# gabeur/mmt

Hardware: AMD Instinct MI355X
Metric: video-text pairs/sec (fwd+bwd+Adam), MSRVTT 7-expert d512 L4 (higher is better)
Workload: dtype bf16; 1 GPU; configs[1]: MSRVTT jsfusion shape, 7 experts x 30 tokens, d512, L4, H4, I3072, batch 32/GPU, dropout 0.1, train mode, Adam; text tower replaced by synthetic (B,768) vectors; global_batch=32, seq_len=218, parallelism=dp1, hip_graphs=True, inputs=resident in HBM, input_slots=8, input_format=dense fp32 dict, text_tower=synthetic, grad_sync=single, grad_wire_dtype=fp32, grad_algo=allreduce, comm_log=False, collectives_captured=False, dense_rows=6976, full=False

## Files before the change

### mmt_amd/csrc/gemm.hip

```cpp
#include "mmt_common.h"
#include "../../include/mmt_hip.h"

#define BK 64

template <int R>
__device__ __forceinline__ void stage_nt(const bf16_t* __restrict__ G, int64_t ld, int row0, int k0,
                                         bf16_t* lds_tile, int wave, int lane) {
#pragma unroll
  for (int i = 0; i < R / 32; ++i) {
    const int rbase = (wave * (R / 32) + i) * 8;
    const int r = rbase + (lane >> 3);
    const int c = (lane & 7) ^ (r & 7);
    const bf16_t* src = G + (int64_t)(row0 + r) * ld + k0 + c * 8;
    __builtin_amdgcn_global_load_lds(GLB_PTR(src), LDS_PTR(lds_tile + rbase * BK), 16, 0, 0);
  }
}

template <int BM, int BN, int EPI>
__global__ __launch_bounds__(256, 2) void gemm_nt_kernel(
    const bf16_t* __restrict__ A, int64_t lda, const bf16_t* __restrict__ B, int64_t ldb,
    void* __restrict__ Cout, int64_t ldc, int M, int N, int K, MmtEpilogue epi,
    const int32_t* __restrict__ n_rows_dev) {
  constexpr int MI = BM / 32, NI = BN / 32;
  __shared__ __attribute__((aligned(16))) bf16_t smem[2 * (BM + BN) * BK];
// ... 234 lines not shown
      const int k2 = k0 + wn * 64 + j * 16 + lg * 4;
      *(f32x4*)(out + (int64_t)n * K2 + k2) = acc[i][j];
    }
  }
}

__device__ __forceinline__ void tr_frag_issue(u32x2& lo, u32x2& hi, unsigned addr) {
  asm volatile("ds_read_b64_tr_b16 %0, %1" : "=v"(lo) : "v"(addr));
  asm volatile("ds_read_b64_tr_b16 %0, %1 offset:4096" : "=v"(hi) : "v"(addr));
}
__device__ __forceinline__ unsigned tr_frag_offset(int ks, int colbase, int lane) {
  const int t = lane & 15, g = lane >> 4;
  const int col = colbase + 4 * (t & 3);
  const int r0 = ks * 32 + 4 * g + (t >> 2);
  const int ch = col >> 3, w = col & 7;
  return (unsigned)((r0 * 128 + ((ch ^ ((r0 & 7) << 1)) << 3) + w) * 2);
}
#define TR_TIE4(x) "+v"(x[0]), "+v"(x[1]), "+v"(x[2]), "+v"(x[3])
__device__ __forceinline__ bf16x8_t tr_join(const u32x2& lo, const u32x2& hi) {
  const u32x4 v = {lo[0], lo[1], hi[0], hi[1]};
  return __builtin_bit_cast(bf16x8_t, v);
}

#ifdef MMT_GEMM2_INSTR
__device__ long long* g_wgrad_dbg = nullptr;
extern "C" int mmt_debug_set_wgrad_buffer(void* p) {
  return (int)hipMemcpyToSymbol(HIP_SYMBOL(g_wgrad_dbg), &p, sizeof(p));
}
#define WTICK(acc) do { const long long tn_ = clock64(); acc += tn_ - tp; tp = tn_; } while (0)
#else
#define WTICK(acc) do {} while (0)
#endif

__global__ __launch_bounds__(512) void wgrad_phased_kernel(MmtWgradGroup g) {
  extern __shared__ __attribute__((aligned(16))) unsigned char wg_smem[];
#ifdef MMT_GEMM2_INSTR
  const long long t_entry = clock64();
#endif
  bf16_t* smem = (bf16_t*)wg_smem;
  const int id = xcd_remap(blockIdx.x, gridDim.x);
  int p = 0;
#pragma unroll 1
  for (int q = 1; q < g.count; ++q)
    if (id >= g.item[q].tile_begin) p = q;
  const MmtWgradItem& it = g.item[p];
  const bf16_t* __restrict__ A = (const bf16_t*)it.A;
  const bf16_t* __restrict__ B = (const bf16_t*)it.B;
  const int64_t lda = it.lda, ldb = it.ldb;
  const int nsplit = it.splits > 1 ? it.splits : 1;
  const int tile = (id - it.tile_begin) / nsplit, split = (id - it.tile_begin) % nsplit;
  const int tiles_k = it.K2 / 128;
  int tn, tk;
  {
    const int PN = it.reserved2 >> 16, PK = it.reserved2 & 0xffff;
    if (PN > 0 && PK > 0) {
      const int per = PN * PK, patches_k = tiles_k / PK;
      const int patch = tile / per, within = tile % per;
      tn = (patch / patches_k) * PN + within / PK;
      tk = (patch % patches_k) * PK + within % PK;
    } else {
      tn = tile / tiles_k;
      tk = tile % tiles_k;
    }
  }
  const int n0 = tn * 128, k0 = tk * 128;
  const int nrows = it.reserved > 0 ? it.reserved
                    : it.n_rows_dev ? min(*it.n_rows_dev, g.rows)
                                    : (g.n_rows_dev ? min(*g.n_rows_dev, g.rows) : g.rows);
  const int units_all = (nrows + 63) / 64;
  const int per_split = (units_all + nsplit - 1) / nsplit;
  const int u0 = split * per_split;
  const int units = max(0, min(units_all, u0 + per_split) - u0);

  const int tid = threadIdx.x, lane = tid & 63, wave8 = tid >> 6;
  const int kg = wave8 >> 2, wave = wave8 & 3;
  const int wk = wave >> 1, wt = wave & 1;
  const int li = lane & 15, lg = lane >> 4;
// ... 224 lines not shown
  constexpr int kWgrad3MinRows = 2048, kWgrad3MinTiles = 192;
  {
    int t3 = 0;
    bool ok = h.rows >= kWgrad3MinRows;
    for (int q = 0; q < h.count && ok; ++q) {
      const MmtWgradItem& it = h.item[q];
      ok = it.A && it.B && it.out && it.N > 0 && it.K2 > 0 && it.N % 256 == 0 && it.K2 % 256 == 0 && it.splits <= 1 &&
           !(it.lda % 8) && !(it.ldb % 8) && !((uintptr_t)it.A & 15) && !((uintptr_t)it.B & 15) && !((uintptr_t)it.out & 15) &&
           it.lda >= 256 && it.ldb >= 256;
      t3 += (it.N / 256) * (it.K2 / 256);
    }
    if (ok && t3 >= kWgrad3MinTiles) {
      int tb = 0;
      for (int q = 0; q < h.count; ++q) {
        MmtWgradItem& it = h.item[q];
        if (it.N_out <= 0 || it.N_out > it.N) it.N_out = it.N;
        if (it.K2_out <= 0 || it.K2_out > it.K2) it.K2_out = it.K2;
        if (it.ldo <= 0) it.ldo = it.K2_out;
        it.tile_begin = tb;
        tb += (it.N / 256) * (it.K2 / 256);
      }
      return mmt_wgrad3_launch(h, tb, (hipStream_t)stream);
    }
  }
  for (int q = 0; q < h.count; ++q) {
    MmtWgradItem& it = h.item[q];
    if (!it.A || !it.B || !it.out || it.N <= 0 || it.K2 <= 0 || it.N % 128 || it.K2 % 128) return MMT_ERR_ARG;
    if ((it.lda % 8) || (it.ldb % 8) || ((uintptr_t)it.A & 15) || ((uintptr_t)it.B & 15) || ((uintptr_t)it.out & 15))
      return MMT_ERR_ALIGN;
    if (it.N_out <= 0 || it.N_out > it.N) it.N_out = it.N;
    if (it.K2_out <= 0 || it.K2_out > it.K2) it.K2_out = it.K2;
    if (it.ldo <= 0) it.ldo = it.K2_out;
    if (it.splits > 1 && (!it.slab || (it.bias_out && !it.bias_slab))) return MMT_ERR_ARG;
    it.tile_begin = tiles;
    tiles += (it.N / 128) * (it.K2 / 128) * (it.splits > 1 ? it.splits : 1);
    {
      const int tn_all = it.N / 128, tk_all = it.K2 / 128;
      int pn = 1, pk = 1;
      for (int c = 1; c <= 8; ++c)
        if (tn_all % c == 0) pn = c;
      for (int c = 1; c <= 32 / pn; ++c)
        if (tk_all % c == 0) pk = c;
      it.reserved2 = (pn << 16) | pk;
    }
  }
  constexpr int lds = 36 * 256 * 16;
  static bool configured = false;
  if (!configured) {
    hipError_t rc = hipFuncSetAttribute((const void*)wgrad_phased_kernel, hipFuncAttributeMaxDynamicSharedMemorySize, lds);
    if (rc != hipSuccess) return (int)rc;
    configured = true;
  }
  hipLaunchKernelGGL(wgrad_phased_kernel, dim3(tiles), dim3(512), lds, (hipStream_t)stream, h);
  return (int)hipGetLastError();
}

__global__ void reduce_slabs_kernel(const float* __restrict__ ws, int splits, int64_t count4,
                                    float* __restrict__ out, int accumulate) {
  for (int64_t i = blockIdx.x * (int64_t)blockDim.x + threadIdx.x; i < count4;
       i += (int64_t)gridDim.x * blockDim.x) {
    f32x4 s = ((const f32x4*)ws)[i];
    for (int k = 1; k < splits; ++k) s += ((const f32x4*)ws)[k * count4 + i];
    if (accumulate) s += ((const f32x4*)out)[i];
    ((f32x4*)out)[i] = s;
  }
}
// ... 151 lines not shown
```

### mmt_amd/csrc/gemm2.hip

```cpp
#include "mmt_common.h"
#include "../../include/mmt_hip.h"
#include "gemm_epi.h"

#define BK 64
template <int ROWS, int NW>
__device__ __forceinline__ void stage2(const bf16_t* __restrict__ G, int64_t ld, int row0, int row_max, int k0,
                                       bf16_t* lds_tile, int wave, int lane) {
  constexpr int PER = ROWS / 8 / NW;
#pragma unroll
  for (int i = 0; i < PER; ++i) {
    const int rbase = (wave * PER + i) * 8;
    const int r = rbase + (lane >> 3);
    const int c = (lane & 7) ^ ((r >> 1) & 7);
    const int gr = min(row0 + r, row_max);
    const bf16_t* src = G + (int64_t)gr * ld + k0 + c * 8;
    __builtin_amdgcn_global_load_lds(GLB_PTR(src), LDS_PTR(lds_tile + rbase * BK), 16, 0, 0);
  }
}

template <int BN> __device__ __forceinline__ int swz_kn(int r) {
  return BN == 128 ? (((r & 7) << 1) | ((r >> 3) & 1)) : ((r >> 1) & 7);
}
template <int BN, int NW>
__device__ __forceinline__ void stage2_kn(const bf16_t* __restrict__ G, int64_t ld, int k0, int n0, bf16_t* lds_tile,
// ... 5 lines not shown
    const int rbase = (wave * PER + i) * RPI;
    const int r = rbase + lane / CHN;
    const int c = (lane % CHN) ^ swz_kn<BN>(r);
    const bf16_t* src = G + (int64_t)(k0 + r) * ld + n0 + c * 8;
    __builtin_amdgcn_global_load_lds(GLB_PTR(src), LDS_PTR(lds_tile + rbase * BN), 16, 0, 0);
  }
}
template <int BN>
__device__ __forceinline__ bf16x8_t frag_kn(const bf16_t* tile, int kk, int colbase, int lane) {
  const int t = lane & 15;
  const int col = colbase + ((lane >> 4) & 1) * 16 + 4 * (t & 3);
  const int r0 = kk * 16 + (lane >> 5) * 8 + (t >> 2), r1 = r0 + 4;
  const int ch = col >> 3, w = col & 7;
  const bf16_t* p0 = tile + r0 * BN + ((ch ^ swz_kn<BN>(r0)) << 3) + w;
  const bf16_t* p1 = tile + r1 * BN + ((ch ^ swz_kn<BN>(r1)) << 3) + w;
  bf16x4_t lo = __builtin_amdgcn_ds_read_tr16_b64_v4bf16((__attribute__((address_space(3))) bf16x4_t*)LDS_PTR(p0));
  bf16x4_t hi = __builtin_amdgcn_ds_read_tr16_b64_v4bf16((__attribute__((address_space(3))) bf16x4_t*)LDS_PTR(p1));
  return __builtin_shufflevector(lo, hi, 0, 1, 2, 3, 4, 5, 6, 7);
}

template <int N>
__device__ __forceinline__ void wait_vmcnt() {
  asm volatile("s_waitcnt vmcnt(%0)" ::"n"(N) : "memory");
}

template <int BM, int BN, int WGM, int WGN, int NS, int EPI, bool BKN = false, bool PH = false>
__device__ __forceinline__ void gemm2_body(
    const bf16_t* __restrict__ A, int64_t lda, const bf16_t* __restrict__ B, int64_t ldb,
    void* __restrict__ Cout, int64_t ldc, int M, int N, int K, const MmtEpilogue& epi,
    const int32_t* __restrict__ n_rows_dev, const int bid, const int nblk) {
  constexpr int GW = WGM * WGN;
  constexpr int NW = PH ? 2 * GW : GW, NT = NW * 64, WTM = BM / WGM, WTN = BN / WGN, MI = WTM / 32, NJ = WTN / 32;
  static_assert(!PH || NS == 4, "the phased loop runs on a four-deep ring");
  constexpr bool STAG = !PH && NW == 8 && NS >= 3;
#ifdef MMT_GEMM2_INSTR
  const long long t_entry = clock64(), w_entry = wall_clock64();
#endif
  extern __shared__ __attribute__((aligned(16))) unsigned char smem_raw[];
  bf16_t* smem = (bf16_t*)smem_raw;

  const int tiles_n = N / BN;
  const int nrows = n_rows_dev ? *n_rows_dev : M;
  const int tid = threadIdx.x;
  const int live_tiles = min(nblk, ((min(nrows, M) + BM - 1) / BM) * tiles_n);
  if (bid >= live_tiles) {
    if constexpr (EPI == MMT_EPI_DGELU) {
      if (epi.colsum && BM >= 128 && bid < ((M + BM - 1) / BM) * tiles_n) {
        const int dm0 = (bid / tiles_n) * BM, dn0 = (bid % tiles_n) * BN;
        for (int h = 0; h < BM / 128; ++h)
          if (dm0 + h * 128 < M && tid < BN) epi.colsum[(int64_t)(dm0 / 128 + h) * N + dn0 + tid] = 0.f;
      }
    }
    return;
  }
  const int id = xcd_remap(bid, live_tiles);
  int tm, tn;
  if (tiles_n * BN >= 1024) {
    constexpr int GROUP = 8;
    const int tile_rows = live_tiles / tiles_n;
    const int band = id / (GROUP * tiles_n), first = band * GROUP;
    const int rows_here = min(GROUP, tile_rows - first);
    const int within = id - band * GROUP * tiles_n;
    tm = first + within % rows_here;
    tn = within / rows_here;
  } else {
    tm = id / tiles_n;
// ... 36 lines not shown
      stage2<BM, NW>(A, lda, m0, amax, s0 * BK, smem + s0 * STAGE, wave, lane);
      if constexpr (BKN) stage2_kn<BN, NW>(B, ldb, s0 * BK, n0, smem + s0 * STAGE + BM * BK, wave, lane);
      else stage2<BN, NW>(B, ldb, n0, bmax, s0 * BK, smem + s0 * STAGE + BM * BK, wave, lane);
    }
  }
  int aoff[MI], boff[NJ], asw[MI], bsw[NJ];
#pragma unroll
  for (int i = 0; i < MI; ++i) {
    const int r = wm * WTM + i * 32 + l31;
    aoff[i] = r * BK; asw[i] = (r >> 1) & 7;
  }
#pragma unroll
  for (int j = 0; j < NJ; ++j) {
    const int r = wn * WTN + j * 32 + l31;
    boff[j] = BM * BK + r * BK; bsw[j] = (r >> 1) & 7;
  }
  int cur = 0;
#ifdef MMT_GEMM2_INSTR
  long long t_wait = 0, t_bar = 0, t_issue = 0, t_comp = 0, t0 = clock64(), tp = t0;
#define TICK(acc) do { const long long tn_ = clock64(); acc += tn_ - tp; tp = tn_; } while (0)
#else
#define TICK(acc) do {} while (0)
#endif
  for (int kt = 0; kt < KT; ++kt) {
    bool do_issue = false;
    int nxt = 0;
    if constexpr (PH) {
      const bool mine = (kt & 1) == kg;
      if (mine) {
        if (kt + 2 < KT) wait_vmcnt<L>();
        else wait_vmcnt<0>();
      }
      TICK(t_wait);
      asm volatile("" ::: "memory");
      __builtin_amdgcn_s_barrier();
      asm volatile("" ::: "memory");
      TICK(t_bar);
      cur = kt % NS;
      if (!mine) {
        issue_ph(kt + NS - 1);
        TICK(t_issue);
        continue;
      }
    } else {
    const int ahead = min(KT - kt - 1, NS - 2);
    if (NS >= 4 && ahead >= 2) wait_vmcnt<2 * L>();
    else if (NS >= 3 && ahead >= 1) wait_vmcnt<L>();
    else wait_vmcnt<0>();
    TICK(t_wait);
    __builtin_amdgcn_s_barrier();
    asm volatile("" ::: "memory");
    TICK(t_bar);
    nxt = cur + NS - 1;
    if (nxt >= NS) nxt -= NS;
    do_issue = kt + NS - 1 < KT;
    }
    if (do_issue && !late_issue) {
      stage2<BM, NW>(A, lda, m0, amax, (kt + NS - 1) * BK, smem + nxt * STAGE, wave, lane);
      if constexpr (BKN) stage2_kn<BN, NW>(B, ldb, (kt + NS - 1) * BK, n0, smem + nxt * STAGE + BM * BK, wave, lane);
      else stage2<BN, NW>(B, ldb, n0, bmax, (kt + NS - 1) * BK, smem + nxt * STAGE + BM * BK, wave, lane);
    }
    TICK(t_issue);
    const bf16_t* st = smem + cur * STAGE;
    if constexpr (PH) {
      static_assert(!BKN, "phased mode: NT operand form");
// ... 14 lines not shown
#pragma unroll
      for (int kk = 0; kk < 4; ++kk) {
        constexpr int PER = MI + NJ;
        if (kk == 0) asm volatile("s_waitcnt lgkmcnt(%0)" ::"n"(3 * PER) : "memory");
        if (kk == 1) asm volatile("s_waitcnt lgkmcnt(%0)" ::"n"(2 * PER) : "memory");
        if (kk == 2) asm volatile("s_waitcnt lgkmcnt(%0)" ::"n"(1 * PER) : "memory");
        if (kk == 3) asm volatile("s_waitcnt lgkmcnt(0)" ::: "memory");
#pragma unroll
        for (int i = 0; i < MI; ++i) asm volatile("" : "+v"(pa[kk][i]));
#pragma unroll
        for (int j = 0; j < NJ; ++j) asm volatile("" : "+v"(pb[kk][j]));
#pragma unroll
        for (int i = 0; i < MI; ++i)
#pragma unroll
          for (int j = 0; j < NJ; ++j)
            acc[i][j] = __builtin_amdgcn_mfma_f32_32x32x16_bf16(__builtin_bit_cast(bf16x8_t, pb[kk][j]),
                                                                __builtin_bit_cast(bf16x8_t, pa[kk][i]), acc[i][j], 0, 0, 0);
        __builtin_amdgcn_sched_barrier(0);
      }
#ifdef MMT_GEMM2_INSTR
      asm volatile("s_nop 0" ::"v"(acc[0][0][0]), "v"(acc[MI - 1][NJ - 1][15]));
#endif
      TICK(t_comp);
      continue;
    }
    bf16x8_t af[2][MI], bfr[2][NJ];
#pragma unroll
    for (int i = 0; i < MI; ++i) af[0][i] = *(const bf16x8_t*)(st + aoff[i] + ((lh ^ asw[i]) << 3));
#pragma unroll
    for (int j = 0; j < NJ; ++j) {
      if constexpr (BKN) bfr[0][j] = frag_kn<BN>(st + BM * BK, 0, wn * WTN + j * 32, lane);
      else bfr[0][j] = *(const bf16x8_t*)(st + boff[j] + ((lh ^ bsw[j]) << 3));
    }
#pragma unroll
    for (int kk = 0; kk < 4; ++kk) {
      if (kk < 3) {
        const int c = (kk + 1) * 2 + lh;
#pragma unroll
        for (int i = 0; i < MI; ++i) af[(kk + 1) & 1][i] = *(const bf16x8_t*)(st + aoff[i] + ((c ^ asw[i]) << 3));
#pragma unroll
        for (int j = 0; j < NJ; ++j) {
          if constexpr (BKN) bfr[(kk + 1) & 1][j] = frag_kn<BN>(st + BM * BK, kk + 1, wn * WTN + j * 32, lane);
          else bfr[(kk + 1) & 1][j] = *(const bf16x8_t*)(st + boff[j] + ((c ^ bsw[j]) << 3));
        }
      }
#pragma unroll
      for (int i = 0; i < MI; ++i)
#pragma unroll
        for (int j = 0; j < NJ; ++j)
          acc[i][j] = __builtin_amdgcn_mfma_f32_32x32x16_bf16(bfr[kk & 1][j], af[kk & 1][i], acc[i][j], 0, 0, 0);
    }
    if (do_issue && late_issue) {
      stage2<BM, NW>(A, lda, m0, amax, (kt + NS - 1) * BK, smem + nxt * STAGE, wave, lane);
      if constexpr (BKN) stage2_kn<BN, NW>(B, ldb, (kt + NS - 1) * BK, n0, smem + nxt * STAGE + BM * BK, wave, lane);
      else stage2<BN, NW>(B, ldb, n0, bmax, (kt + NS - 1) * BK, smem + nxt * STAGE + BM * BK, wave, lane);
    }
    if constexpr (!PH) cur = cur + 1 == NS ? 0 : cur + 1;
#ifdef MMT_GEMM2_INSTR
    asm volatile("s_nop 0" ::"v"(acc[0][0][0]), "v"(acc[MI - 1][NJ - 1][15]));
#endif
    TICK(t_comp);
  }
  if constexpr (PH) wait_vmcnt<0>();
#ifdef MMT_GEMM2_INSTR
  const long long t_loop_end = clock64();
#endif

#ifdef MMT_GEMM2_INSTR
  long long eticks[3] = {0, 0, 0};
  gemm_tile_epilogue<BM, BN, WGM, WGN, NT, EPI, PH>(acc, smem_raw, m0, n0, M, N, nrows, Cout, ldc, epi, wm, wn, kg, tid, eticks);
  const long long e_head = eticks[2] - t_loop_end, e_stage = eticks[0], e_sweep = eticks[1];
#else
  gemm_tile_epilogue<BM, BN, WGM, WGN, NT, EPI, PH>(acc, smem_raw, m0, n0, M, N, nrows, Cout, ldc, epi, wm, wn, kg, tid, nullptr);
#endif
#ifdef MMT_GEMM2_INSTR
  if (epi.row_index == nullptr && epi.seed_dev != nullptr && tid == 0) {
    long long* dbgbuf = (long long*)epi.seed_dev + (int64_t)bid * 16;
    dbgbuf[0] = t_wait; dbgbuf[1] = t_bar; dbgbuf[2] = t_issue; dbgbuf[3] = t_comp;
    dbgbuf[4] = t_loop_end - t0; dbgbuf[5] = clock64() - t_loop_end; dbgbuf[7] = KT;
    dbgbuf[8] = t0 - t_entry; dbgbuf[9] = e_head; dbgbuf[10] = e_stage; dbgbuf[11] = e_sweep; dbgbuf[12] = w_entry;
    asm volatile("s_waitcnt vmcnt(0)" ::: "memory");
    dbgbuf[6] = clock64() - t_entry;
    dbgbuf[13] = wall_clock64();
    dbgbuf[14] = (long long)__builtin_amdgcn_s_getreg((31 << 11) | 20);
    dbgbuf[15] = (long long)__builtin_amdgcn_s_getreg((31 << 11) | 4);
  }
#endif
}

template <int BM, int BN, int WGM, int WGN, int NS, int EPI, bool BKN = false, bool PH = false>
__global__ __launch_bounds__((PH ? 2 : 1) * WGM * WGN * 64) void gemm2_kernel(
    const bf16_t* __restrict__ A, int64_t lda, const bf16_t* __restrict__ B, int64_t ldb,
    void* __restrict__ Cout, int64_t ldc, int M, int N, int K, MmtEpilogue epi,
    const int32_t* __restrict__ n_rows_dev) {
  gemm2_body<BM, BN, WGM, WGN, NS, EPI, BKN, PH>(A, lda, B, ldb, Cout, ldc, M, N, K, epi, n_rows_dev, (int)blockIdx.x,
                                                 (int)gridDim.x);
// ... 318 lines not shown
```

### mmt_amd/csrc/gemm_epi.h

```cpp
#pragma once
#include "mmt_common.h"
#include "../../include/mmt_hip.h"
#include "gelu_lut.h"

typedef __attribute__((ext_vector_type(16))) float f32x16;

__device__ __forceinline__ float gelu_lut_abs(const float* __restrict__ lut, unsigned b) {
  const unsigned mag = b & 0x7fffu;
  const unsigned idx = min(max(mag, (unsigned)MMT_GELU_LUT_LO), (unsigned)(MMT_GELU_LUT_LO + MMT_GELU_LUT_N - 1)) - MMT_GELU_LUT_LO;
  return lut[idx];
}
__device__ __forceinline__ float gelu_lut(const float* __restrict__ lut, unsigned b) {
  const float t = gelu_lut_abs(lut, b);
  return bf2f((bf16_t)b) * ((b & 0x8000u) ? 1.0f - t : t);
}
__device__ __forceinline__ float gelu_grad_lut(const float* __restrict__ lut, unsigned b) {
  const float t = gelu_lut_abs(lut, b);
  return (b & 0x8000u) ? 1.0f - t : t;
}

template <int BM, int BN, int WGM, int WGN, int NT, int EPI, bool PH>
__device__ __forceinline__ void gemm_tile_epilogue(f32x16 (&acc)[BM / WGM / 32][BN / WGN / 32], unsigned char* smem_raw, int m0, int n0,
                                                   int M, int N, int nrows, void* __restrict__ Cout, int64_t ldc,
                                                   const MmtEpilogue& epi, int wm, int wn, int kg, int tid, long long* ticks) {
  constexpr int WTM = BM / WGM, WTN = BN / WGN, MI = WTM / 32, NJ = WTN / 32;
  constexpr int P = BN + 4;
  constexpr int CB = (NT * 4) % BN == 0 ? BN : 64;
  constexpr int NCB = BN / CB;
  constexpr int CG = CB / 4;
  constexpr int RG = NT / CG;
  constexpr int CH = BM < 64 ? BM : 64;
  static_assert(BN % CB == 0 && NT % CG == 0 && CH % RG == 0, "epilogue geometry");
  const int lane = tid & 63, l31 = lane & 31, lh = lane >> 5;
  float* st = (float*)smem_raw;
  float* red = st + CH * P;
  const int cg = tid % CG, rg = tid / CG;
  f32x4 bias4[NCB];
#pragma unroll
  for (int cb = 0; cb < NCB; ++cb) {
    bias4[cb] = (f32x4){0.f, 0.f, 0.f, 0.f};
    if constexpr (EPI == MMT_EPI_BIAS_BF16 || EPI == MMT_EPI_BIAS_GELU || EPI == MMT_EPI_BIAS_DROP_RES ||
                  EPI == MMT_EPI_BIAS_F32)
      bias4[cb] = *(const f32x4*)(epi.bias + n0 + cb * CB + cg * 4);
  }
  unsigned dkey = 0;
  if constexpr (EPI == MMT_EPI_BIAS_DROP_RES) dkey = eff_key(epi.drop_key, epi.seed_dev);
  float csum[NCB][4];
#pragma unroll
  for (int cb = 0; cb < NCB; ++cb) csum[cb][0] = csum[cb][1] = csum[cb][2] = csum[cb][3] = 0.f;
  const int64_t rb = m0 + rg, cb0 = n0 + cg * 4;
  const int64_t off_c = rb * ldc + cb0, off_res = rb * epi.ldres + cb0, off_aux = rb * epi.ldaux + cb0,
                off_o2 = rb * epi.ldout2 + cb0, off_dot = rb * epi.lddot + cb0;
  constexpr int SW = CH / RG, NPF = (BM / CH) * SW * NCB;
  constexpr bool PF_FITS = NPF <= 8;
  constexpr bool PFC = !PF_FITS && SW * NCB <= 8;
  constexpr bool PF_RES = PF_FITS && (EPI == MMT_EPI_BIAS_DROP_RES || EPI == MMT_EPI_ADD_F32);
  constexpr bool PF_AUX = PF_FITS && (EPI == MMT_EPI_DGELU || EPI == MMT_EPI_BF16);
  f32x4 pf_res[PF_RES ? NPF : 1];
  u32x2 pf_aux[PF_AUX ? NPF : 1];
  int pf_orow[PF_RES && EPI == MMT_EPI_BIAS_DROP_RES ? (BM / CH) * SW : 1];
  if constexpr (PF_RES || PF_AUX) {
#pragma unroll
    for (int ch = 0; ch < BM / CH; ++ch)
#pragma unroll
      for (int sw = 0; sw < SW; ++sw) {
        const int dr = ch * CH + sw * RG;
        const bool in = m0 + dr + rg < M;
        const int row = in ? m0 + dr + rg : M - 1;
        if constexpr (PF_RES && EPI == MMT_EPI_BIAS_DROP_RES)
          pf_orow[ch * SW + sw] = (epi.drop_thr16 && epi.row_index) ? epi.row_index[row] : row;
#pragma unroll
        for (int cb = 0; cb < NCB; ++cb) {
          if constexpr (PF_RES) {
            const int64_t o = in ? off_res + (int64_t)dr * epi.ldres + cb * CB : (int64_t)(M - 1) * epi.ldres + cb0 + cb * CB;
            pf_res[(ch * SW + sw) * NCB + cb] = *(const f32x4*)(epi.res + o);
          }
          if constexpr (PF_AUX && EPI == MMT_EPI_DGELU) {
            const int64_t o = in ? off_aux + (int64_t)dr * epi.ldaux + cb * CB : (int64_t)(M - 1) * epi.ldaux + cb0 + cb * CB;
            pf_aux[(ch * SW + sw) * NCB + cb] = *(const u32x2*)((const bf16_t*)epi.aux + o);
          }
          if constexpr (PF_AUX && EPI == MMT_EPI_BF16) {
            if (epi.dot_out) {
              const int64_t o = in ? off_dot + (int64_t)dr * epi.lddot + cb * CB : (int64_t)(M - 1) * epi.lddot + cb0 + cb * CB;
              pf_aux[(ch * SW + sw) * NCB + cb] = *(const u32x2*)((const bf16_t*)epi.dot_src + o);
            }
          }
        }
      }
  }
  constexpr bool LUT = EPI == MMT_EPI_BIAS_GELU || EPI == MMT_EPI_DGELU;
  constexpr int LUTN = (MMT_GELU_LUT_N + NT - 1) / NT;
  float* lut = red + RG * BN;
  float lutv[LUT ? LUTN : 1];
  if constexpr (LUT) {
    const float* src = EPI == MMT_EPI_BIAS_GELU ? g_gelu_lut_cdf : g_gelu_lut_dgelu;
#pragma unroll
    for (int i = 0; i < LUTN; ++i) lutv[i] = src[min(i * NT + tid, MMT_GELU_LUT_N - 1)];
  }
  __syncthreads();
  if constexpr (LUT) {
#pragma unroll
    for (int i = 0; i < LUTN; ++i)
      if (i * NT + tid < MMT_GELU_LUT_N) lut[i * NT + tid] = lutv[i];
  }
#ifdef MMT_GEMM2_INSTR
  long long e_stage = 0, e_sweep = 0, tp = clock64();
  const long long e_t0 = tp;
#define ETICK(acc) do { const long long tn_ = clock64(); acc += tn_ - tp; tp = tn_; } while (0)
#else
#define ETICK(acc) do {} while (0)
#endif
#pragma unroll
// ... 154 lines not shown
```

### mmt_amd/csrc/texthead2.hip

```cpp
#include "mmt_common.h"
#include "../../include/mmt_hip.h"
#include "video_front.h"

typedef __attribute__((ext_vector_type(16))) float f32x16;

#define TH_W 16
#define TH_T (64 * TH_W)
#define TH_TMAX 8

struct ThArgs {
  MmtTextHeads h;
  const float* text; const float* text_moe;
  float* ws;
  float* text_embds; float* text_weights;
  const float* de; const float* tw; const float* dtw;
  float* dtext_moe;
  int N, C, M, d, K, use_bn, training;
  uint32_t drop_key, thr16; float drop_scale;
  const uint32_t* seed_dev; uint32_t* key_dev; long long* nbt;
};

struct ThWs { float *y, *x1, *mean, *rstd, *dyg, *dz, *dlogit, *sg, *o, *part; };
__host__ __device__ inline ThWs th_layout(float* ws, int N, int M, int d) {
  const int64_t nmd = (int64_t)N * M * d, md = (int64_t)M * d;
// ... 29 lines not shown
    }
  }
  f32x16 acc;
#pragma unroll
  for (int r = 0; r < 16; ++r) acc[r] = 0.f;
#pragma unroll
  for (int t = 0; t < TH_TMAX; ++t) {
    if (kbeg + 8 * t < kend) {
#pragma unroll
      for (int u = 0; u < 4; ++u) acc = __builtin_amdgcn_mfma_f32_32x32x2f32(av[t][u], bv[t][u], acc, 0, 0, 0);
    }
  }
  return acc;
}

__device__ __forceinline__ float splitk_reduce(ThSmem& sm, const f32x16& acc, int wave, int lane) {
#pragma unroll
  for (int r = 0; r < 16; ++r) sm.red[wave][r][lane] = acc[r];
  __syncthreads();
  float v = 0.f;
#pragma unroll
  for (int w = 0; w < TH_W; ++w) v += sm.red[w][wave][lane];
  return v;
}
__device__ __forceinline__ int tile_row(int wave, int lane) { return (wave & 3) + 8 * (wave >> 2) + 4 * (lane >> 5); }

__device__ __forceinline__ float half_wave_sum(float v) {
#pragma unroll
  for (int s = 16; s > 0; s >>= 1) v += __shfl_xor(v, s, 64);
  return v;
}

__device__ __forceinline__ int k_slice(int K) { return (((K + TH_W - 1) / TH_W) + 7) & ~7; }

__device__ __forceinline__ f32x4 moe_input4(const ThArgs& a, unsigned key, int n, int k4) {
  if (a.text_moe) return *(const f32x4*)(a.text_moe + (int64_t)n * a.K + k4);
  f32x4 v = *(const f32x4*)(a.text + (int64_t)n * a.K + k4);
  if (a.thr16) {
    bool kp[4];
    keep4(key, (unsigned long long)n * (unsigned)a.K + (unsigned)k4, a.thr16, kp);
#pragma unroll
    for (int e = 0; e < 4; ++e) v[e] = kp[e] ? v[e] * a.drop_scale : 0.f;
  }
  return v;
}

// ... 213 lines not shown
    const float t = lane < a.M ? a.tw[(int64_t)n * a.M + lane] : 0.f, dv = lane < a.M ? a.dtw[(int64_t)n * a.M + lane] : 0.f;
    const float dot = wave_sum(t * dv);
    if (lane < a.M) {
      dl[lane] = t * (dv - dot);
      w.dlogit[(int64_t)n * a.M + lane] = dl[lane];
    }
  }
  __syncthreads();
  if (!a.dtext_moe) return;
  const unsigned key = (!a.text_moe && a.thr16 && a.key_dev) ? *a.key_dev : 0u;
  for (int k4 = tid * 4; k4 < a.K; k4 += 1024) {
    f32x4 s = {0.f, 0.f, 0.f, 0.f};
    for (int m = 0; m < a.M; ++m) s += *(const f32x4*)(a.h.moe_w[m] + k4) * dl[m];
    if (!a.text_moe && a.thr16) {
      bool kp[4];
      keep4(key, (unsigned long long)n * (unsigned)a.K + (unsigned)k4, a.thr16, kp);
#pragma unroll
      for (int e = 0; e < 4; ++e) s[e] = kp[e] ? s[e] * a.drop_scale : 0.f;
    }
    *(f32x4*)(a.dtext_moe + (int64_t)n * a.K + k4) = s;
  }
}

__device__ __forceinline__ f32x16 mm_tn_tile(const float (*T)[33], const float* __restrict__ G, int64_t ldg, int N, int l31,
                                             int h) {
  float b[16];
#pragma unroll
  for (int kk = 0; kk < 16; ++kk) {
    const int k = 2 * kk + h;
    b[kk] = k < N ? G[(int64_t)k * ldg + l31] : 0.f;
  }
  f32x16 acc;
#pragma unroll
  for (int r = 0; r < 16; ++r) acc[r] = 0.f;
#pragma unroll
  for (int kk = 0; kk < 16; ++kk) acc = __builtin_amdgcn_mfma_f32_32x32x2f32(T[2 * kk + h][l31], b[kk], acc, 0, 0, 0);
  return acc;
}
__device__ __forceinline__ void store_tile(const f32x16& acc, float* __restrict__ out, int64_t ldo, int l31, int h) {
#pragma unroll
  for (int r = 0; r < 16; ++r) out[(int64_t)((r & 3) + 8 * (r >> 2) + 4 * h) * ldo + l31] = acc[r];
}

__global__ __launch_bounds__(TH_T) void th_bwd2_kernel(ThArgs a) {
  extern __shared__ __attribute__((aligned(16))) unsigned char th_smem_raw[];
  ThSmem& sm = *(ThSmem*)th_smem_raw;
  const int tid = threadIdx.x, lane = tid & 63, wave = tid >> 6, l31 = lane & 31, h = lane >> 5;
  const int ct = a.d / 32;
  const int m = blockIdx.x / ct, j0 = (blockIdx.x % ct) * 32;
  const ThWs w = th_layout(a.ws, a.N, a.M, a.d);
  const int n = tid >> 5, j = tid & 31, col = j0 + j;
  const int64_t p = ((int64_t)n * a.M + m) * a.d + col;
  const bool live = n < a.N;
  const float dzv = live ? w.dz[p] : 0.f;
  float dx = dzv;
  if (a.use_bn) {
    const float mu = w.mean[(int64_t)m * a.d + col], rs = w.rstd[(int64_t)m * a.d + col], ga = a.h.bn_gamma[m][col];
    const float xh = live ? (w.x1[p] - mu) * rs : 0.f;
    sm.tile[0][n][j] = dzv;
    sm.tile[1][n][j] = dzv * xh;
    __syncthreads();
    {
      const int r = tid & 31, c = tid >> 5;
      const float s1 = half_wave_sum(sm.tile[0][r][c]), s2 = half_wave_sum(sm.tile[1][r][c]);
      if (r == 0) {
        sm.colv[0][c] = s1;
        sm.colv[1][c] = s2;
        if (a.h.g_bn_beta[m]) a.h.g_bn_beta[m][j0 + c] = s1;
        if (a.h.g_bn_gamma[m]) a.h.g_bn_gamma[m][j0 + c] = s2;
      }
    }
    __syncthreads();
    if (a.training) dx = ga * rs * (dzv - sm.colv[0][j] / a.N - xh * sm.colv[1][j] / a.N);
    else dx = ga * rs * dzv;
    if (!live) dx = 0.f;
  }
  if (live) w.dz[p] = dx;
  sm.tile[2][n][j] = dx;
  __syncthreads();
  {
    const float sb = half_wave_sum(sm.tile[2][tid & 31][tid >> 5]);
    if ((tid & 31) == 0 && a.h.g_b2[m]) a.h.g_b2[m][j0 + (tid >> 5)] = sb;
  }
  if (a.h.g_w2[m]) {
    for (int c_t = wave; c_t < ct; c_t += TH_W) {
      const f32x16 acc = mm_tn_tile(sm.tile[2], w.y + (int64_t)m * a.d + c_t * 32, (int64_t)a.M * a.d, a.N, l31, h);
      store_tile(acc, a.h.g_w2[m] + (int64_t)j0 * a.d + c_t * 32, a.d, l31, h);
    }
  }
}

__global__ __launch_bounds__(TH_T) void th_bwd3_kernel(ThArgs a) {
  extern __shared__ __attribute__((aligned(16))) unsigned char th_smem_raw[];
  ThSmem& sm = *(ThSmem*)th_smem_raw;
  const int tid = threadIdx.x, lane = tid & 63, wave = tid >> 6, l31 = lane & 31, h = lane >> 5;
  const int ct = a.d / 32, gemm_blocks = a.M * ct;
  const ThWs w = th_layout(a.ws, a.N, a.M, a.d);
  if ((int)blockIdx.x >= gemm_blocks) {
    const int kb_n = (a.K + 4 * TH_T - 1) / (4 * TH_T);
    const int q = blockIdx.x - gemm_blocks, m = q / kb_n, k4 = ((q % kb_n) * TH_T + tid) * 4;
    const unsigned key = (!a.text_moe && a.thr16 && a.key_dev) ? *a.key_dev : 0u;
    if (k4 < a.K && a.h.g_moe_w[m]) {
      f32x4 s = {0.f, 0.f, 0.f, 0.f};
#pragma unroll 8
      for (int n = 0; n < a.N; ++n) s += moe_input4(a, key, n, k4) * w.dlogit[(int64_t)n * a.M + m];
      *(f32x4*)(a.h.g_moe_w[m] + k4) = s;
    }
    if (q % kb_n == 0 && tid == 0 && a.h.g_moe_b[m]) {
      float s = 0.f;
      for (int n = 0; n < a.N; ++n) s += w.dlogit[(int64_t)n * a.M + m];
      a.h.g_moe_b[m][0] = s;
    }
    return;
  }
  const int m = blockIdx.x / ct, j0 = (blockIdx.x % ct) * 32;
  const int per = k_slice(a.d), kbeg = wave * per, kend = min(a.d, kbeg + per);
  {
    const float* ap = w.dz + ((int64_t)min(l31, a.N - 1) * a.M + m) * a.d;
    const bool iok = l31 < a.N;
    const float* bp = a.h.w2[m] + j0 + l31;
    f32x4 av[TH_TMAX], bv[TH_TMAX];
#pragma unroll
    for (int t = 0; t < TH_TMAX; ++t) {
      const int k0 = kbeg + 8 * t + 4 * h;
      av[t] = bv[t] = (f32x4){0.f, 0.f, 0.f, 0.f};
      if (k0 + 3 < kend) {
        if (iok) av[t] = *(const f32x4*)(ap + k0);
#pragma unroll
        for (int u = 0; u < 4; ++u) bv[t][u] = bp[(int64_t)(k0 + u) * a.d];
      }
    }
    f32x16 acc;
#pragma unroll
    for (int r = 0; r < 16; ++r) acc[r] = 0.f;
#pragma unroll
    for (int t = 0; t < TH_TMAX; ++t) {
      if (kbeg + 8 * t < kend) {
#pragma unroll
        for (int u = 0; u < 4; ++u) acc = __builtin_amdgcn_mfma_f32_32x32x2f32(av[t][u], bv[t][u], acc, 0, 0, 0);
      }
    }
    float v = splitk_reduce(sm, acc, wave, lane);
    const int n = tile_row(wave, lane);
    if (n < a.N) {
      const int64_t p = ((int64_t)n * a.M + m) * a.d + j0 + l31;
      v += w.dyg[p];
      w.dyg[p] = v;
    } else {
      v = 0.f;
    }
    sm.tile[2][n][l31] = v;
  }
  __syncthreads();
  {
    const float sb = half_wave_sum(sm.tile[2][tid & 31][tid >> 5]);
    if ((tid & 31) == 0 && a.h.g_b1[m]) a.h.g_b1[m][j0 + (tid >> 5)] = sb;
  }
  if (a.h.g_w1[m]) {
    const int kt_n = a.K / 32;
    for (int kt = wave; kt < kt_n; kt += TH_W) {
      const f32x16 acc = mm_tn_tile(sm.tile[2], a.text + kt * 32, a.K, a.N, l31, h);
      store_tile(acc, a.h.g_w1[m] + (int64_t)j0 * a.K + kt * 32, a.K, l31, h);
    }
  }
}

extern "C" int mmt_text_heads_fast(int N, int M, int d, int K) {
  return N >= 1 && N <= 32 && M >= 1 && M <= MMT_MAX_EXPERTS && d % 32 == 0 && d >= 32 && d <= 1024 && K % 32 == 0 &&
         K >= 32 && K <= 1024;
}

static int th_configure() {
  static bool done = false;
  if (done) return 0;
  const void* fns[] = {(const void*)th_fwd1_kernel, (const void*)th_fwd2_kernel, (const void*)th_bwd2_kernel,
                       (const void*)th_bwd3_kernel, (const void*)th_fwd1_plan_kernel, (const void*)th_fwd2_cast_kernel};
  for (const void* f : fns) {
    hipError_t rc = hipFuncSetAttribute(f, hipFuncAttributeMaxDynamicSharedMemorySize, (int)sizeof(ThSmem));
    if (rc != hipSuccess) return (int)rc;
  }
  done = true;
  return 0;
}

static void th_fill(ThArgs& a, const MmtTextHeads* h, const float* text, const float* text_moe, int N, int C, int M, int d,
                    int K, int use_bn, int training, float* ws, const MmtTextHeadsOpts* o) {
// ... 76 lines not shown
```

Baseline: 24810 pairs/s.

## Prefetch epilogue operands during GEMM tail, sort wgrad items, hoist text-head loads

Three unrelated changes. The phased GEMM now issues its epilogue bias, residual and aux loads during the last NS-1 k-steps, widening the vmcnt waits so these loads overlap the remaining MMA work. The wgrad launcher sorts items by row-unit length when lengths differ and remaps XCD placement per item, so long tiles dispatch first and load imbalance drops. The text-head backward kernels load their TN-GEMM operands before the split-k reduction barrier to hide global latency, at the cost of more registers, and they unroll the tile loop to at most two tiles per wave.

```diff
diff --git a/mmt_amd/csrc/gemm.hip b/mmt_amd/csrc/gemm.hip
--- a/mmt_amd/csrc/gemm.hip
+++ b/mmt_amd/csrc/gemm.hip
@@ -280,6 +280,7 @@
   return __builtin_bit_cast(bf16x8_t, v);
 }
 
+#define WGRAD_LISTED (1 << 30)
 #ifdef MMT_GEMM2_INSTR
 __device__ long long* g_wgrad_dbg = nullptr;
 extern "C" int mmt_debug_set_wgrad_buffer(void* p) {
@@ -296,7 +297,8 @@
   const long long t_entry = clock64();
 #endif
   bf16_t* smem = (bf16_t*)wg_smem;
-  const int id = xcd_remap(blockIdx.x, gridDim.x);
+  const bool listed = (g.item[0].reserved2 & WGRAD_LISTED) != 0;
+  const int id = listed ? (int)blockIdx.x : xcd_remap(blockIdx.x, gridDim.x);
   int p = 0;
 #pragma unroll 1
   for (int q = 1; q < g.count; ++q)
@@ -306,11 +308,12 @@
   const bf16_t* __restrict__ B = (const bf16_t*)it.B;
   const int64_t lda = it.lda, ldb = it.ldb;
   const int nsplit = it.splits > 1 ? it.splits : 1;
-  const int tile = (id - it.tile_begin) / nsplit, split = (id - it.tile_begin) % nsplit;
   const int tiles_k = it.K2 / 128;
+  const int local = listed ? xcd_remap(id - it.tile_begin, (it.N / 128) * tiles_k * nsplit) : id - it.tile_begin;
+  const int tile = local / nsplit, split = local % nsplit;
   int tn, tk;
   {
-    const int PN = it.reserved2 >> 16, PK = it.reserved2 & 0xffff;
+    const int PN = (it.reserved2 >> 16) & 0xff, PK = it.reserved2 & 0xffff;
     if (PN > 0 && PK > 0) {
       const int per = PN * PK, patches_k = tiles_k / PK;
       const int patch = tile / per, within = tile % per;
@@ -581,6 +584,22 @@
       }
       return mmt_wgrad3_launch(h, tb, (hipStream_t)stream);
     }
+  }
+  bool listed = false;
+  {
+    int len[MMT_WGRAD_MAX];
+    for (int q = 0; q < h.count; ++q) {
+      const MmtWgradItem& it = h.item[q];
+      const int rows_q = it.reserved > 0 ? it.reserved : h.rows, sp = it.splits > 1 ? it.splits : 1;
+      len[q] = ((rows_q + 63) / 64 + sp - 1) / sp;
+      listed = listed || len[q] != len[0];
+    }
+    if (listed)
+      for (int q = 1; q < h.count; ++q)
+        for (int r = q; r > 0 && len[r] > len[r - 1]; --r) {
+          const MmtWgradItem ti = h.item[r]; h.item[r] = h.item[r - 1]; h.item[r - 1] = ti;
+          const int tl = len[r]; len[r] = len[r - 1]; len[r - 1] = tl;
+        }
   }
   for (int q = 0; q < h.count; ++q) {
     MmtWgradItem& it = h.item[q];
@@ -600,7 +619,7 @@
         if (tn_all % c == 0) pn = c;
       for (int c = 1; c <= 32 / pn; ++c)
         if (tk_all % c == 0) pk = c;
-      it.reserved2 = (pn << 16) | pk;
+      it.reserved2 = (pn << 16) | pk | (listed ? WGRAD_LISTED : 0);
     }
   }
   constexpr int lds = 36 * 256 * 16;
diff --git a/mmt_amd/csrc/gemm2.hip b/mmt_amd/csrc/gemm2.hip
--- a/mmt_amd/csrc/gemm2.hip
+++ b/mmt_amd/csrc/gemm2.hip
@@ -51,6 +51,22 @@
 template <int N>
 __device__ __forceinline__ void wait_vmcnt() {
   asm volatile("s_waitcnt vmcnt(%0)" ::"n"(N) : "memory");
+}
+template <int N>
+__device__ __forceinline__ void wait_vmcnt_plus(int extra) {
+  static_assert(N + 9 < 64, "vmcnt is a 6-bit counter");
+  switch (extra) {
+    case 1: wait_vmcnt<N + 1>(); break;
+    case 2: wait_vmcnt<N + 2>(); break;
+    case 3: wait_vmcnt<N + 3>(); break;
+    case 4: wait_vmcnt<N + 4>(); break;
+    case 5: wait_vmcnt<N + 5>(); break;
+    case 6: wait_vmcnt<N + 6>(); break;
+    case 7: wait_vmcnt<N + 7>(); break;
+    case 8: wait_vmcnt<N + 8>(); break;
+    case 9: wait_vmcnt<N + 9>(); break;
+    default: wait_vmcnt<N>(); break;
+  }
 }
 
 template <int BM, int BN, int WGM, int WGN, int NS, int EPI, bool BKN = false, bool PH = false>
@@ -71,6 +87,8 @@
   const int tiles_n = N / BN;
   const int nrows = n_rows_dev ? *n_rows_dev : M;
   const int tid = threadIdx.x;
+  EpiOperands<BM, BN, NT, EPI> eops;
+  if constexpr (PH) eops.load_seed(epi);
   const int live_tiles = min(nblk, ((min(nrows, M) + BM - 1) / BM) * tiles_n);
   if (bid >= live_tiles) {
     if constexpr (EPI == MMT_EPI_DGELU) {
@@ -153,14 +171,14 @@
 #else
 #define TICK(acc) do {} while (0)
 #endif
-  for (int kt = 0; kt < KT; ++kt) {
+  auto kstep = [&](const int kt, const int pf_vm) __attribute__((always_inline)) {
     bool do_issue = false;
     int nxt = 0;
     if constexpr (PH) {
       const bool mine = (kt & 1) == kg;
       if (mine) {
-        if (kt + 2 < KT) wait_vmcnt<L>();
-        else wait_vmcnt<0>();
+        if (kt + 2 < KT) wait_vmcnt_plus<L>(pf_vm);
+        else wait_vmcnt_plus<0>(pf_vm);
       }
       TICK(t_wait);
       asm volatile("" ::: "memory");
@@ -171,7 +189,7 @@
       if (!mine) {
         issue_ph(kt + NS - 1);
         TICK(t_issue);
-        continue;
+        return;
       }
     } else {
     const int ahead = min(KT - kt - 1, NS - 2);
@@ -232,7 +250,7 @@
       asm volatile("s_nop 0" ::"v"(acc[0][0][0]), "v"(acc[MI - 1][NJ - 1][15]));
 #endif
       TICK(t_comp);
-      continue;
+      return;
     }
     bf16x8_t af[2][MI], bfr[2][NJ];
 #pragma unroll
@@ -270,18 +288,25 @@
     asm volatile("s_nop 0" ::"v"(acc[0][0][0]), "v"(acc[MI - 1][NJ - 1][15]));
 #endif
     TICK(t_comp);
-  }
-  if constexpr (PH) wait_vmcnt<0>();
+  };
+  const int kt_pf = !PH ? KT : KT > NS - 1 ? KT - (NS - 1) : 0;
+  for (int kt = 0; kt < kt_pf; ++kt) kstep(kt, 0);
+  if constexpr (PH) {
+    eops.load(m0, n0, M, epi, tid);
+    const int pf_vm = EpiOperands<BM, BN, NT, EPI>::vm_ops(epi);
+    for (int kt = kt_pf; kt < KT; ++kt) kstep(kt, pf_vm);
+    wait_vmcnt<0>();
+  }
 #ifdef MMT_GEMM2_INSTR
   const long long t_loop_end = clock64();
 #endif
 
 #ifdef MMT_GEMM2_INSTR
   long long eticks[3] = {0, 0, 0};
-  gemm_tile_epilogue<BM, BN, WGM, WGN, NT, EPI, PH>(acc, smem_raw, m0, n0, M, N, nrows, Cout, ldc, epi, wm, wn, kg, tid, eticks);
+  gemm_tile_epilogue<BM, BN, WGM, WGN, NT, EPI, PH>(acc, smem_raw, m0, n0, M, N, nrows, Cout, ldc, epi, wm, wn, kg, tid, eticks, PH ? &eops : nullptr);
   const long long e_head = eticks[2] - t_loop_end, e_stage = eticks[0], e_sweep = eticks[1];
 #else
-  gemm_tile_epilogue<BM, BN, WGM, WGN, NT, EPI, PH>(acc, smem_raw, m0, n0, M, N, nrows, Cout, ldc, epi, wm, wn, kg, tid, nullptr);
+  gemm_tile_epilogue<BM, BN, WGM, WGN, NT, EPI, PH>(acc, smem_raw, m0, n0, M, N, nrows, Cout, ldc, epi, wm, wn, kg, tid, nullptr, PH ? &eops : nullptr);
 #endif
 #ifdef MMT_GEMM2_INSTR
   if (epi.row_index == nullptr && epi.seed_dev != nullptr && tid == 0) {
diff --git a/mmt_amd/csrc/gemm_epi.h b/mmt_amd/csrc/gemm_epi.h
--- a/mmt_amd/csrc/gemm_epi.h
+++ b/mmt_amd/csrc/gemm_epi.h
@@ -19,10 +19,89 @@
   return (b & 0x8000u) ? 1.0f - t : t;
 }
 
+template <int BM, int BN, int NT, int EPI>
+struct EpiOperands {
+  static constexpr int CB = (NT * 4) % BN == 0 ? BN : 64, NCB = BN / CB, CG = CB / 4, RG = NT / CG, CH = BM < 64 ? BM : 64;
+  static constexpr int SW = CH / RG, NPF = (BM / CH) * SW * NCB;
+  static constexpr bool FITS = NPF <= 8;
+  static constexpr bool RES = FITS && (EPI == MMT_EPI_BIAS_DROP_RES || EPI == MMT_EPI_ADD_F32);
+  static constexpr bool AUX = FITS && (EPI == MMT_EPI_DGELU || EPI == MMT_EPI_BF16);
+  f32x4 res[RES ? NPF : 1];
+  u32x2 aux[AUX ? NPF : 1];
+  int orow[RES && EPI == MMT_EPI_BIAS_DROP_RES ? (BM / CH) * SW : 1];
+  static constexpr bool BIAS = EPI == MMT_EPI_BIAS_BF16 || EPI == MMT_EPI_BIAS_GELU || EPI == MMT_EPI_BIAS_DROP_RES ||
+                               EPI == MMT_EPI_BIAS_F32;
+  f32x4 bias[NCB];
+  unsigned seed;
+  __device__ __forceinline__ void load_seed(const MmtEpilogue& epi) {
+    seed = 0;
+    if constexpr (EPI == MMT_EPI_BIAS_DROP_RES)
+      if (epi.seed_dev) seed = *epi.seed_dev;
+  }
+  __device__ __forceinline__ unsigned key(const MmtEpilogue& epi) const {
+    if constexpr (EPI != MMT_EPI_BIAS_DROP_RES) return 0;
+    return epi.seed_dev ? mix32(epi.drop_key ^ mix32(seed + 0x632be5abU)) : epi.drop_key;
+  }
+  static __device__ __forceinline__ int vm_ops(const MmtEpilogue& epi) {
+    int n = BIAS ? NCB : 0;
+    if constexpr (RES) n += NPF;
+    if constexpr (RES && EPI == MMT_EPI_BIAS_DROP_RES) n += (epi.drop_thr16 && epi.row_index) ? (BM / CH) * SW : 0;
+    if constexpr (AUX && EPI == MMT_EPI_DGELU) n += NPF;
+    if constexpr (AUX && EPI == MMT_EPI_BF16) n += epi.dot_out ? NPF : 0;
+    return n;
+  }
+  __device__ __forceinline__ void load_bias(int n0, const MmtEpilogue& epi, int tid) {
+#pragma unroll
+    for (int cb = 0; cb < NCB; ++cb) {
+      bias[cb] = (f32x4){0.f, 0.f, 0.f, 0.f};
+      if constexpr (BIAS) bias[cb] = *(const f32x4*)(epi.bias + n0 + cb * CB + (tid % CG) * 4);
+    }
+  }
+  __device__ __forceinline__ void load(int m0, int n0, int M, const MmtEpilogue& epi, int tid) {
+    load_bias(n0, epi, tid);
+    load_rows(m0, n0, M, epi, tid);
+  }
+  __device__ __forceinline__ void load_rows(int m0, int n0, int M, const MmtEpilogue& epi, int tid) {
+    if constexpr (RES || AUX) {
+      const int cg = tid % CG, rg = tid / CG;
+      const int64_t rb = m0 + rg, cb0 = n0 + cg * 4;
+      const int64_t off_res = rb * epi.ldres + cb0, off_aux = rb * epi.ldaux + cb0, off_dot = rb * epi.lddot + cb0;
+#pragma unroll
+      for (int ch = 0; ch < BM / CH; ++ch)
+#pragma unroll
+        for (int sw = 0; sw < SW; ++sw) {
+          const int dr = ch * CH + sw * RG;
+          const bool in = m0 + dr + rg < M;
+          const int row = in ? m0 + dr + rg : M - 1;
+          if constexpr (RES && EPI == MMT_EPI_BIAS_DROP_RES)
+            orow[ch * SW + sw] = (epi.drop_thr16 && epi.row_index) ? epi.row_index[row] : row;
+#pragma unroll
+          for (int cb = 0; cb < NCB; ++cb) {
+            if constexpr (RES) {
+              const int64_t o = in ? off_res + (int64_t)dr * epi.ldres + cb * CB : (int64_t)(M - 1) * epi.ldres + cb0 + cb * CB;
+              res[(ch * SW + sw) * NCB + cb] = *(const f32x4*)(epi.res + o);
+            }
+            if constexpr (AUX && EPI == MMT_EPI_DGELU) {
+              const int64_t o = in ? off_aux + (int64_t)dr * epi.ldaux + cb * CB : (int64_t)(M - 1) * epi.ldaux + cb0 + cb * CB;
+              aux[(ch * SW + sw) * NCB + cb] = *(const u32x2*)((const bf16_t*)epi.aux + o);
+            }
+            if constexpr (AUX && EPI == MMT_EPI_BF16) {
+              if (epi.dot_out) {
+                const int64_t o = in ? off_dot + (int64_t)dr * epi.lddot + cb * CB : (int64_t)(M - 1) * epi.lddot + cb0 + cb * CB;
+                aux[(ch * SW + sw) * NCB + cb] = *(const u32x2*)((const bf16_t*)epi.dot_src + o);
+              }
+            }
+          }
+        }
+    }
+  }
+};
+
 template <int BM, int BN, int WGM, int WGN, int NT, int EPI, bool PH>
 __device__ __forceinline__ void gemm_tile_epilogue(f32x16 (&acc)[BM / WGM / 32][BN / WGN / 32], unsigned char* smem_raw, int m0, int n0,
                                                    int M, int N, int nrows, void* __restrict__ Cout, int64_t ldc,
-                                                   const MmtEpilogue& epi, int wm, int wn, int kg, int tid, long long* ticks) {
+                                                   const MmtEpilogue& epi, int wm, int wn, int kg, int tid, long long* ticks,
+                                                   EpiOperands<BM, BN, NT, EPI>* ops_loaded = nullptr) {
   constexpr int WTM = BM / WGM, WTN = BN / WGN, MI = WTM / 32, NJ = WTN / 32;
   constexpr int P = BN + 4;
   constexpr int CB = (NT * 4) % BN == 0 ? BN : 64;
@@ -35,59 +114,28 @@
   float* st = (float*)smem_raw;
   float* red = st + CH * P;
   const int cg = tid % CG, rg = tid / CG;
-  f32x4 bias4[NCB];
-#pragma unroll
-  for (int cb = 0; cb < NCB; ++cb) {
-    bias4[cb] = (f32x4){0.f, 0.f, 0.f, 0.f};
-    if constexpr (EPI == MMT_EPI_BIAS_BF16 || EPI == MMT_EPI_BIAS_GELU || EPI == MMT_EPI_BIAS_DROP_RES ||
-                  EPI == MMT_EPI_BIAS_F32)
-      bias4[cb] = *(const f32x4*)(epi.bias + n0 + cb * CB + cg * 4);
-  }
-  unsigned dkey = 0;
-  if constexpr (EPI == MMT_EPI_BIAS_DROP_RES) dkey = eff_key(epi.drop_key, epi.seed_dev);
   float csum[NCB][4];
 #pragma unroll
   for (int cb = 0; cb < NCB; ++cb) csum[cb][0] = csum[cb][1] = csum[cb][2] = csum[cb][3] = 0.f;
   const int64_t rb = m0 + rg, cb0 = n0 + cg * 4;
   const int64_t off_c = rb * ldc + cb0, off_res = rb * epi.ldres + cb0, off_aux = rb * epi.ldaux + cb0,
                 off_o2 = rb * epi.ldout2 + cb0, off_dot = rb * epi.lddot + cb0;
-  constexpr int SW = CH / RG, NPF = (BM / CH) * SW * NCB;
-  constexpr bool PF_FITS = NPF <= 8;
+  using Ops = EpiOperands<BM, BN, NT, EPI>;
+  constexpr int SW = Ops::SW;
+  constexpr bool PF_FITS = Ops::FITS, PF_RES = Ops::RES, PF_AUX = Ops::AUX;
   constexpr bool PFC = !PF_FITS && SW * NCB <= 8;
-  constexpr bool PF_RES = PF_FITS && (EPI == MMT_EPI_BIAS_DROP_RES || EPI == MMT_EPI_ADD_F32);
-  constexpr bool PF_AUX = PF_FITS && (EPI == MMT_EPI_DGELU || EPI == MMT_EPI_BF16);
-  f32x4 pf_res[PF_RES ? NPF : 1];
-  u32x2 pf_aux[PF_AUX ? NPF : 1];
-  int pf_orow[PF_RES && EPI == MMT_EPI_BIAS_DROP_RES ? (BM / CH) * SW : 1];
-  if constexpr (PF_RES || PF_AUX) {
-#pragma unroll
-    for (int ch = 0; ch < BM / CH; ++ch)
-#pragma unroll
-      for (int sw = 0; sw < SW; ++sw) {
-        const int dr = ch * CH + sw * RG;
-        const bool in = m0 + dr + rg < M;
-        const int row = in ? m0 + dr + rg : M - 1;
-        if constexpr (PF_RES && EPI == MMT_EPI_BIAS_DROP_RES)
-          pf_orow[ch * SW + sw] = (epi.drop_thr16 && epi.row_index) ? epi.row_index[row] : row;
-#pragma unroll
-        for (int cb = 0; cb < NCB; ++cb) {
-          if constexpr (PF_RES) {
-            const int64_t o = in ? off_res + (int64_t)dr * epi.ldres + cb * CB : (int64_t)(M - 1) * epi.ldres + cb0 + cb * CB;
-            pf_res[(ch * SW + sw) * NCB + cb] = *(const f32x4*)(epi.res + o);
-          }
-          if constexpr (PF_AUX && EPI == MMT_EPI_DGELU) {
-            const int64_t o = in ? off_aux + (int64_t)dr * epi.ldaux + cb * CB : (int64_t)(M - 1) * epi.ldaux + cb0 + cb * CB;
-            pf_aux[(ch * SW + sw) * NCB + cb] = *(const u32x2*)((const bf16_t*)epi.aux + o);
-          }
-          if constexpr (PF_AUX && EPI == MMT_EPI_BF16) {
-            if (epi.dot_out) {
-              const int64_t o = in ? off_dot + (int64_t)dr * epi.lddot + cb * CB : (int64_t)(M - 1) * epi.lddot + cb0 + cb * CB;
-              pf_aux[(ch * SW + sw) * NCB + cb] = *(const u32x2*)((const bf16_t*)epi.dot_src + o);
-            }
-          }
-        }
-      }
-  }
+  Ops ops_own;
+  if (!ops_loaded) {
+    ops_own.load_bias(n0, epi, tid);
+    ops_own.load_seed(epi);
+  }
+  Ops& ops = ops_loaded ? *ops_loaded : ops_own;
+  auto& bias4 = ops.bias;
+  const unsigned dkey = ops.key(epi);
+  if (!ops_loaded) ops_own.load_rows(m0, n0, M, epi, tid);
+  auto& pf_res = ops.res;
+  auto& pf_aux = ops.aux;
+  auto& pf_orow = ops.orow;
   constexpr bool LUT = EPI == MMT_EPI_BIAS_GELU || EPI == MMT_EPI_DGELU;
   constexpr int LUTN = (MMT_GELU_LUT_N + NT - 1) / NT;
   float* lut = red + RG * BN;
diff --git a/mmt_amd/csrc/texthead2.hip b/mmt_amd/csrc/texthead2.hip
--- a/mmt_amd/csrc/texthead2.hip
+++ b/mmt_amd/csrc/texthead2.hip
@@ -75,6 +75,16 @@
 #pragma unroll
   for (int w = 0; w < TH_W; ++w) v += sm.red[w][wave][lane];
   return v;
+}
+__device__ __forceinline__ float splitk_reduce_then(ThSmem& sm, const f32x16& acc, int wave, int lane, float last) {
+#pragma clang fp reassociate(off)
+#pragma unroll
+  for (int r = 0; r < 16; ++r) sm.red[wave][r][lane] = acc[r];
+  __syncthreads();
+  float v = sm.red[TH_W - 2][wave][lane] + sm.red[TH_W - 1][wave][lane];
+#pragma unroll
+  for (int w = TH_W - 3; w >= 0; --w) v = v + sm.red[w][wave][lane];
+  return v + last;
 }
 __device__ __forceinline__ int tile_row(int wave, int lane) { return (wave & 3) + 8 * (wave >> 2) + 4 * (lane >> 5); }
 
@@ -334,14 +344,15 @@
   }
 }
 
-__device__ __forceinline__ f32x16 mm_tn_tile(const float (*T)[33], const float* __restrict__ G, int64_t ldg, int N, int l31,
-                                             int h) {
-  float b[16];
+__device__ __forceinline__ void tn_load(float (&b)[16], const float* __restrict__ G, int64_t ldg, int N, int l31, int h) {
 #pragma unroll
   for (int kk = 0; kk < 16; ++kk) {
     const int k = 2 * kk + h;
-    b[kk] = k < N ? G[(int64_t)k * ldg + l31] : 0.f;
-  }
+    const float g = G[(int64_t)min(k, N - 1) * ldg + l31];
+    b[kk] = k < N ? g : 0.f;
+  }
+}
+__device__ __forceinline__ f32x16 tn_mma(const float (*T)[33], const float (&b)[16], int l31, int h) {
   f32x16 acc;
 #pragma unroll
   for (int r = 0; r < 16; ++r) acc[r] = 0.f;
@@ -366,6 +377,10 @@
   const bool live = n < a.N;
   const float dzv = live ? w.dz[p] : 0.f;
   float dx = dzv;
+  const bool gw2 = a.h.g_w2[m] != nullptr;
+  float yb0[16], yb1[16];
+  if (gw2 && wave < ct) tn_load(yb0, w.y + (int64_t)m * a.d + wave * 32, (int64_t)a.M * a.d, a.N, l31, h);
+  if (gw2 && wave + TH_W < ct) tn_load(yb1, w.y + (int64_t)m * a.d + (wave + TH_W) * 32, (int64_t)a.M * a.d, a.N, l31, h);
   if (a.use_bn) {
     const float mu = w.mean[(int64_t)m * a.d + col], rs = w.rstd[(int64_t)m * a.d + col], ga = a.h.bn_gamma[m][col];
     const float xh = live ? (w.x1[p] - mu) * rs : 0.f;
@@ -394,11 +409,10 @@
     const float sb = half_wave_sum(sm.tile[2][tid & 31][tid >> 5]);
     if ((tid & 31) == 0 && a.h.g_b2[m]) a.h.g_b2[m][j0 + (tid >> 5)] = sb;
   }
-  if (a.h.g_w2[m]) {
-    for (int c_t = wave; c_t < ct; c_t += TH_W) {
-      const f32x16 acc = mm_tn_tile(sm.tile[2], w.y + (int64_t)m * a.d + c_t * 32, (int64_t)a.M * a.d, a.N, l31, h);
-      store_tile(acc, a.h.g_w2[m] + (int64_t)j0 * a.d + c_t * 32, a.d, l31, h);
-    }
+  if (gw2) {
+    if (wave < ct) store_tile(tn_mma(sm.tile[2], yb0, l31, h), a.h.g_w2[m] + (int64_t)j0 * a.d + wave * 32, a.d, l31, h);
+    if (wave + TH_W < ct)
+      store_tile(tn_mma(sm.tile[2], yb1, l31, h), a.h.g_w2[m] + (int64_t)j0 * a.d + (wave + TH_W) * 32, a.d, l31, h);
   }
 }
 
@@ -427,6 +441,9 @@
   }
   const int m = blockIdx.x / ct, j0 = (blockIdx.x % ct) * 32;
   const int per = k_slice(a.d), kbeg = wave * per, kend = min(a.d, kbeg + per);
+  const bool gw1 = a.h.g_w1[m] != nullptr;
+  const int kt_n = a.K / 32;
+  float tb0[16], tb1[16];
   {
     const float* ap = w.dz + ((int64_t)min(l31, a.N - 1) * a.M + m) * a.d;
     const bool iok = l31 < a.N;
@@ -452,11 +469,13 @@
         for (int u = 0; u < 4; ++u) acc = __builtin_amdgcn_mfma_f32_32x32x2f32(av[t][u], bv[t][u], acc, 0, 0, 0);
       }
     }
-    float v = splitk_reduce(sm, acc, wave, lane);
     const int n = tile_row(wave, lane);
+    const int64_t p = ((int64_t)n * a.M + m) * a.d + j0 + l31;
+    const float dyg0 = n < a.N ? w.dyg[p] : 0.f;
+    if (gw1 && wave < kt_n) tn_load(tb0, a.text + wave * 32, a.K, a.N, l31, h);
+    if (gw1 && wave + TH_W < kt_n) tn_load(tb1, a.text + (wave + TH_W) * 32, a.K, a.N, l31, h);
+    float v = splitk_reduce_then(sm, acc, wave, lane, dyg0);
     if (n < a.N) {
-      const int64_t p = ((int64_t)n * a.M + m) * a.d + j0 + l31;
-      v += w.dyg[p];
       w.dyg[p] = v;
     } else {
       v = 0.f;
@@ -468,12 +487,10 @@
     const float sb = half_wave_sum(sm.tile[2][tid & 31][tid >> 5]);
     if ((tid & 31) == 0 && a.h.g_b1[m]) a.h.g_b1[m][j0 + (tid >> 5)] = sb;
   }
-  if (a.h.g_w1[m]) {
-    const int kt_n = a.K / 32;
-    for (int kt = wave; kt < kt_n; kt += TH_W) {
-      const f32x16 acc = mm_tn_tile(sm.tile[2], a.text + kt * 32, a.K, a.N, l31, h);
-      store_tile(acc, a.h.g_w1[m] + (int64_t)j0 * a.K + kt * 32, a.K, l31, h);
-    }
+  if (gw1) {
+    if (wave < kt_n) store_tile(tn_mma(sm.tile[2], tb0, l31, h), a.h.g_w1[m] + (int64_t)j0 * a.K + wave * 32, a.K, l31, h);
+    if (wave + TH_W < kt_n)
+      store_tile(tn_mma(sm.tile[2], tb1, l31, h), a.h.g_w1[m] + (int64_t)j0 * a.K + (wave + TH_W) * 32, a.K, l31, h);
   }
 }
 
```

After: 25170 pairs/s (median of 6 runs). 1.01x the previous value.
